# myfavouritekk/vdetlib

Measured on AMD Instinct MI355X. Metric: boxes/sec whole-node (NMS+temporal-conv+link), 300f×10k-box synth; mAP parity, higher is better.
Workload: dtype f32; 1 GPU; configs[1]+[2]: 1 video/GPU, 300 frames x 10000 boxes x 200 classes; per-(frame,class) NMS thresh 0.30 + temporal max-pool w=3 + 3-tap temporal convolution; greedy tubelets: 10 tracks/class (stop < 0.90), IoU-link >= 0.50, spatial max-pool IoU > 0.70 + completion + temporal max-pool; frames=300, boxes=10000, classes=200, scores=rand, parallelism=video-per-gpu x1, 4 distinct videos in flight per GPU

## Files before the change

### vdetlib_amd/csrc/graphlists_kernels.hpp

```cpp
#pragma once
#include <hip/hip_runtime.h>
#include <stdint.h>

#include "nms_kernels.hpp"

namespace vdet {

__device__ __forceinline__ int qreach_slot(const GroupDesc &gd, int g) { return ((gd.box_off >> 8) + g) * 4; }

__global__ __launch_bounds__(256) void row_classes_kernel(const float4 *__restrict__ xbox, const GroupDesc *__restrict__ groups,
                                                          const uint32_t *__restrict__ group_flags, float one_minus_t,
                                                          uint16_t *__restrict__ rowperm, float *__restrict__ qreach)
{
    __shared__ float sw[256];
    __shared__ float sreach[256];
    const int g = blockIdx.x, t = blockIdx.y, tid = threadIdx.x;
    if (!(group_flags[g] & kFlagRegular)) return;
    const GroupDesc gd = groups[g];
    if (t * 256 >= gd.nbox) return;
    const int s = t * 256 + tid;
    const bool valid = s < gd.nbox;
    float wd = 3.0e38f, reach = -3.0e38f;
    if (valid) { const float4 b = xbox[gd.box_off + s]; wd = b.z - b.x; reach = b.x + one_minus_t * ((b.z - b.x) + 1.0f) * 1.001f + 1.0f; }
    sw[tid] = wd;
    __syncthreads();
    int rank = 0;
    for (int j = 0; j < 256; ++j) { const float o = sw[j]; rank += (o < wd || (o == wd && j < tid)) ? 1 : 0; }
    if (valid) rowperm[gd.box_off + t * 256 + rank] = (uint16_t)s;
    sreach[rank] = reach;
    __syncthreads();
    float rc = sreach[tid];
#pragma unroll
    for (int d = 32; d > 0; d >>= 1) rc = fmaxf(rc, __shfl_xor(rc, d, 64));
    if ((tid & 63) == 0) qreach[qreach_slot(gd, g) + 4 * t + (tid >> 6)] = rc;
}

struct ListItem { int32_t group; int32_t tq; };

struct GraphListsParams {
    const float4 *xbox;
    const uint16_t *xord;
    const GroupDesc *groups;
    const uint32_t *group_flags;
    const ListItem *items;
    int nitems;
    float t32, one_minus_t;
    uint32_t *row_deg;
    const float2 *reach_table;
    const uint16_t *rowperm;
    const float *qreach;
    uint16_t *adj;
    uint32_t slot_cap;
    int *status;
    int over_bits;
    uint32_t trash_off;
};

__device__ __forceinline__ void emit_half(uint16_t *__restrict__ adj, uint32_t h, uint32_t boff, const uint16_t *ids, uint32_t *lpos,
                                          const uint16_t myid)
{
    constexpr int kSlots = 4;
    if (__ballot(h != 0u) == 0ull) return;
    uint32_t hk[kSlots];
    uint16_t ek[kSlots];
    int bk[kSlots];
#pragma unroll
    for (int k = 0; k < kSlots; ++k) { hk[k] = h; bk[k] = __builtin_ctz(h) & 31; h &= h - 1u; }
#pragma unroll
    for (int k = 0; k < kSlots; ++k) ek[k] = ids[bk[k]];
#pragma unroll
    for (int k = 0; k < kSlots; ++k) {
        if (hk[k] != 0u) {
            *reinterpret_cast<uint16_t *>(reinterpret_cast<char *>(adj) + (boff + 2u * k)) = ek[k];
            const uint32_t o = __hip_atomic_fetch_add(&lpos[bk[k]], 2u, __ATOMIC_RELAXED, __HIP_MEMORY_SCOPE_WAVEFRONT);
            *reinterpret_cast<uint16_t *>(reinterpret_cast<char *>(adj) + o) = myid;
        }
    }
    boff += 2u * kSlots;
    while (__ballot(h != 0u) != 0ull) {
        if (h != 0u) {
            const int b = __builtin_ctz(h);
            *reinterpret_cast<uint16_t *>(reinterpret_cast<char *>(adj) + boff) = ids[b];
            const uint32_t o = __hip_atomic_fetch_add(&lpos[b], 2u, __ATOMIC_RELAXED, __HIP_MEMORY_SCOPE_WAVEFRONT);
            *reinterpret_cast<uint16_t *>(reinterpret_cast<char *>(adj) + o) = myid;
            boff += 2u;
            h &= h - 1u;
        }
    }
}

__device__ __forceinline__ void emit_block(const uint32_t slot_cap, uint16_t *__restrict__ adj, int *__restrict__ status, const int over_bits,
                                           const uint32_t trash_off, unsigned long long m, const uint32_t tcnt, const uint32_t pat,
                                           const uint32_t ptat, const uint32_t row_slot, const uint32_t col_slot, const uint16_t *cids,
                                           const uint16_t myid, uint32_t *lpos, const int lane)
{
    const uint32_t cnt = (uint32_t)__popcll(m);
    const bool rover = pat + cnt > slot_cap, cover = ptat + tcnt > slot_cap;
    if ((rover && cnt) || (cover && tcnt)) atomicOr(status, over_bits);
    lpos[lane] = cover ? trash_off : (col_slot * slot_cap + ptat) * 2u;
    const uint32_t boff = rover ? trash_off : (row_slot * slot_cap + pat) * 2u;
    emit_half(adj, (uint32_t)m, boff, cids, lpos, myid);
    emit_half(adj, (uint32_t)(m >> 32), boff + 2u * (uint32_t)__popc((uint32_t)m), cids + 32, lpos + 32, myid);
}

template <bool XS, bool INTS>
__device__ __forceinline__ void margin_block(const float4 brx, const float rarea, const float4 *sb, const float *sa, float t32, float t_lo,
                                             uint32_t &lo, uint32_t &hi, bool &anyb)
{
    uint32_t nr0 = 0, nq0 = 0, nr1 = 0, nq1 = 0;
#pragma unroll 1
    for (int g = 0; g < 4; ++g) {
#pragma unroll
        for (int j = 0; j < 8; ++j) {
            const int k = 31 - 8 * g - j;
            float mr, mq;
            pred_margins<XS, INTS>(brx, rarea, sb[k], sa[k], t32, t_lo, mr, mq);
            shl1_or_sign(nr0, mr); shl1_or_sign(nq0, mq);
        }
    }
#pragma unroll 1
    for (int g = 0; g < 4; ++g) {
#pragma unroll
        for (int j = 0; j < 8; ++j) {
            const int k = 31 - 8 * g - j;
            float mr, mq;
            pred_margins<XS, INTS>(brx, rarea, sb[32 + k], sa[32 + k], t32, t_lo, mr, mq);
            shl1_or_sign(nr1, mr); shl1_or_sign(nq1, mq);
        }
    }
    lo = ~nr0; hi = ~nr1;
    anyb = (nr0 != nq0) | (nr1 != nq1);
}

__global__ __launch_bounds__(64, 6) void graph_lists_kernel(const GraphListsParams prm)
{
    __shared__ float4 sbox[2][64];
    __shared__ float sarea[2][64];
    __shared__ uint16_t scord[2][64];
    __shared__ uint32_t lpos[64];
    const int per = gridDim.x >> 3;
    const int idx = (blockIdx.x & 7) * per + (blockIdx.x >> 3);
    if (idx >= prm.nitems) return;
    const ListItem it = prm.items[idx];
    const uint32_t gf = prm.group_flags[it.group];
    if (!(gf & kFlagRegular)) return;
    const GroupDesc gd = prm.groups[it.group];
    const int B = gd.nbox, W = (B + 63) >> 6;
    const int lane = threadIdx.x;
    const int mt = it.tq >> 2, qd = it.tq & 3;
    const int s = mt * 256 + qd * 64 + lane;
    const int v = s < B ? (int)prm.rowperm[gd.box_off + s] : B;
    const unsigned long long rowvalid = __ballot(v < B);
    if (rowvalid == 0ull) return;
    const float my_reach = prm.qreach[qreach_slot(gd, it.group) + it.tq];
    const float2 *rtab = prm.reach_table + reach_slot(gd, it.group);
    const float4 *xb = prm.xbox + gd.box_off;
    const uint16_t *xo = prm.xord + gd.box_off;
    const float t32 = prm.t32;
    const float t_lo = t32 * (1.0f - 4.76837158203125e-7f);
    const TransposeConsts tcs = transpose_consts(lane);
    const bool ints = (gf & kFlagU16) != 0u;
    const uint32_t slot_cap = prm.slot_cap;
    uint16_t *adj = prm.adj;

    float4 br = make_float4(0.f, 0.f, 0.f, 0.f);
    uint16_t myid = 0;
    if (v < B) { br = xb[v]; myid = xo[v]; }
    const float rarea = box_area(br);
    float4 brx = br;
    if (ints) { brx.z += 1.0f; brx.w += 1.0f; }

    int c = mt * 4;
    {
        const int u = c * 64 + lane;
        float4 bc = make_float4(0.f, 0.f, 0.f, 0.f);
        uint16_t oc = 0;
        if (u < B) { bc = xb[u]; oc = xo[u]; }
        sarea[0][lane] = box_area(bc);
        if (ints) { bc.z += 1.0f; bc.w += 1.0f; }
        sbox[0][lane] = bc; scord[0][lane] = oc;
    }
    unsigned long long pm = 0ull;
    uint32_t pat = 0u, ptat = 0u, ptcnt = 0u;
    int pc = -1;
    float fnext = (c + 1 < W) ? rtab[c + 1].y : 3.0e38f;
    for (int buf = 0; c < W; ++c, buf ^= 1) {
        const bool dtile = (c >> 2) == mt;
        const int cn = c + 1;
        bool more = cn < W;
        float4 bn = make_float4(0.f, 0.f, 0.f, 0.f);
        uint16_t on = 0;
        const float fn = __uint_as_float(__builtin_amdgcn_readfirstlane(__float_as_uint(fnext)));
        fnext = (c + 2 < W) ? rtab[c + 2].y : 3.0e38f;
        if (more) {
            more = ((cn >> 2) == mt) || fn <= my_reach;
            const int u = cn * 64 + lane;
            if (more && u < B) { bn = xb[u]; on = xo[u]; }
        }
        const int cols_left = B - c * 64;
        const unsigned long long colvalid = cols_left >= 64 ? ~0ull : ((1ull << cols_left) - 1ull);
        uint32_t lo, hi;
        bool anyb;
        if (ints) { if (!dtile) margin_block<true, true>(brx, rarea, sbox[buf], sarea[buf], t32, t_lo, lo, hi, anyb);
                    else margin_block<false, true>(brx, rarea, sbox[buf], sarea[buf], t32, t_lo, lo, hi, anyb); }
        else { if (!dtile) margin_block<true, false>(brx, rarea, sbox[buf], sarea[buf], t32, t_lo, lo, hi, anyb);
               else margin_block<false, false>(brx, rarea, sbox[buf], sarea[buf], t32, t_lo, lo, hi, anyb); }
        if (__builtin_expect(__ballot(anyb) != 0ull, 0)) {
            lo = hi = 0u;
            for (int k = 0; k < 64; ++k) {
                float4 bk = sbox[buf][k];
                if (ints) { bk.z -= 1.0f; bk.w -= 1.0f; }
                const bool p = pair_pred_exact_slow(br, rarea, bk, sarea[buf][k], t32);
                if (k < 32) lo |= p ? (1u << k) : 0u; else hi |= p ? (1u << (k - 32)) : 0u;
            }
        }
        unsigned long long m = (((unsigned long long)hi << 32) | lo) & colvalid;
        if (dtile) {
            const int d = v - c * 64;
            m &= d < 0 ? ~0ull : (d >= 63 ? 0ull : ~((2ull << d) - 1ull));
        }
        if (v >= B) m = 0ull;
        uint32_t tlo = (uint32_t)m, thi = (uint32_t)(m >> 32);
        wave_transpose64(tlo, thi, tcs);
        if (pc >= 0)
            emit_block(slot_cap, adj, prm.status, prm.over_bits, prm.trash_off, pm, ptcnt, pat, ptat, (uint32_t)(gd.box_off + v),
                       (uint32_t)(gd.box_off + pc * 64 + lane), scord[buf ^ 1], myid, lpos, lane);
        {
            unsigned long long tm = 0ull;
            const int u = c * 64 + lane;
            if (u < B) tm = (((unsigned long long)thi << 32) | tlo) & rowvalid;
            const uint32_t cnt = (uint32_t)__popcll(m), tcnt = (uint32_t)__popcll(tm);
            pat = 0u; ptat = 0u;
            if (cnt) pat = atomicAdd(&prm.row_deg[gd.box_off + v], cnt);
            if (tcnt) ptat = atomicAdd(&prm.row_deg[gd.box_off + u], tcnt);
            pm = m; ptcnt = tcnt; pc = c;
        }
        if (!more) break;
        sarea[buf ^ 1][lane] = box_area(bn);
        if (ints) { bn.z += 1.0f; bn.w += 1.0f; }
        sbox[buf ^ 1][lane] = bn; scord[buf ^ 1][lane] = on;
    }
    if (pc >= 0)
        emit_block(slot_cap, adj, prm.status, prm.over_bits, prm.trash_off, pm, ptcnt, pat, ptat, (uint32_t)(gd.box_off + v),
                   (uint32_t)(gd.box_off + pc * 64 + lane), scord[(pc - mt * 4) & 1], myid, lpos, lane);
}

}
```

### vdetlib_amd/csrc/nms_kernels.hpp

```cpp
#pragma once
#include <hip/hip_runtime.h>
#include <stdint.h>

namespace vdet {

struct GroupDesc {
    int32_t box_off;
    int32_t nbox;
    int64_t bits_off;
};

__device__ __host__ __forceinline__ int64_t bit_word(int nbox, int v, int c)
{
    const int W = (nbox + 63) >> 6;
    return ((int64_t)(v >> 6) * W + c) * 64 + (v & 63);
}
__host__ __device__ __forceinline__ int64_t bit_words_of_group(int nbox)
{
    const int64_t W = (nbox + 63) >> 6;
    return W * W * 64;
}

struct TileDesc {
    int32_t group;
// ... 171 lines not shown
        }
        mn = fminf(mn, b.x); mx = fmaxf(mx, b.x); wm = fmaxf(wm, (b.z - b.x) + 1.0f);
    }
    smin[tid] = mn; smax[tid] = mx; swm[tid] = wm;
    for (int i = tid; i < 257; i += 256) hist[i] = 0;
    __syncthreads();
    for (int d = 128; d > 0; d >>= 1) {
        if (tid < d) { smin[tid] = fminf(smin[tid], smin[tid + d]); smax[tid] = fmaxf(smax[tid], smax[tid + d]); swm[tid] = fmaxf(swm[tid], swm[tid + d]); }
        __syncthreads();
    }
    const float xmin = smin[0], xmax = smax[0];
    const float scale = xmax > xmin ? 256.0f / (xmax - xmin) : 0.0f;
    for (int r = tid; r < B; r += 256) atomicAdd(&hist[xbucket(fb[r].x, xmin, scale) + 1], 1u);
    __syncthreads();
    if (tid == 0) {
        uint32_t run = 0;
        for (int k = 0; k <= 256; ++k) { run += hist[k]; cum[(int64_t)f * 257 + k] = run; }
        info[f * 4 + 0] = xmin; info[f * 4 + 1] = scale; info[f * 4 + 2] = swm[0]; info[f * 4 + 3] = 0.0f;
    }
}

__device__ __forceinline__ void xwindow(const FrameIndex &ix, int f, float x1c, float wc, double t, int &r0, int &r1)
{
    const float xmin = ix.info[f * 4 + 0], scale = ix.info[f * 4 + 1], wmax = ix.info[f * 4 + 2];
    const double wj = fmin((double)wmax, (double)wc / t * 1.001);
    const double lo = (double)x1c - (1.0 - t) * wj * 1.001 - 1.0;
    const double hi = (double)x1c + (1.0 - t) * (double)wc * 1.001 + 1.0;
    const int b0 = xbucket((float)fmax(lo, -3.0e38), xmin, scale);
    const int b1 = xbucket((float)fmin(hi, 3.0e38), xmin, scale);
    r0 = (int)ix.cum[(int64_t)f * 257 + b0];
    r1 = (int)ix.cum[(int64_t)f * 257 + b1 + 1];
}

__global__ __launch_bounds__(256) void frame_flags_kernel(const float4 *__restrict__ boxes,
                                                          const GroupDesc *__restrict__ groups,
                                                          uint32_t *__restrict__ group_flags,
                                                          int *__restrict__ n_irregular)
{
    const GroupDesc gd = groups[blockIdx.x];
    int bad = 0, wide = 0;
    const float inf = __uint_as_float(0x7F800000u);
    for (int v = threadIdx.x; v < gd.nbox; v += 256) {
        const float4 b = boxes[gd.box_off + v];
        const float w = (b.z - b.x) + 1.0f, h = (b.w - b.y) + 1.0f;
        const float a = w * h;
        const bool ok = fabsf(b.x) < inf && fabsf(b.y) < inf && fabsf(b.z) < inf && fabsf(b.w) < inf &&
                        w > 0.0f && h > 0.0f && a < inf;
        bad |= ok ? 0 : 1;
        const bool small = b.x == truncf(b.x) && b.y == truncf(b.y) && b.z == truncf(b.z) && b.w == truncf(b.w) &&
                           fmaxf(fmaxf(b.x, b.y), fmaxf(b.z, b.w)) <= 65535.0f &&
                           ((__float_as_uint(b.x) | __float_as_uint(b.y) | __float_as_uint(b.z) | __float_as_uint(b.w)) >> 31) == 0u;
        wide |= small ? 0 : 1;
    }
    const int any_bad = __syncthreads_or(bad);
    const int any_wide = __syncthreads_or(wide);
    if (threadIdx.x == 0) {
        group_flags[blockIdx.x] = (any_bad ? 0u : kFlagRegular) | (any_wide ? 0u : kFlagU16);
        if (any_bad) atomicAdd(n_irregular, 1);
    }
}

__device__ __attribute__((noinline)) bool pair_pred_exact_slow(float4 bi, float iarea, float4 bj, float jarea, float t32)
{
    return (pair_pred(bi, iarea, bj, jarea, t32) & 1u) != 0;
}

struct TilePair {
    int32_t group;
    int16_t rt, ct;
};

__device__ __forceinline__ float amax(float a, float b) { float r; asm("v_max_f32 %0, %1, %2" : "=v"(r) : "v"(a), "v"(b)); return r; }
__device__ __forceinline__ float amin(float a, float b) { float r; asm("v_min_f32 %0, %1, %2" : "=v"(r) : "v"(a), "v"(b)); return r; }

template <bool XSORTED = false>
__device__ __forceinline__ bool pred_regular(float4 br, float rarea, float4 bc, float carea, float t32, float t32e,
                                             bool &border)
{
    const float xx1 = XSORTED ? bc.x : amax(br.x, bc.x);
    const float yy1 = amax(br.y, bc.y);
    const float xx2 = amin(br.z, bc.z);
    const float yy2 = amin(br.w, bc.w);
    const float w = amax(0.0f, (xx2 - xx1) + 1.0f);
    const float h = (yy2 - yy1) + 1.0f;
    const float inter = w * h;
    const float uni = (rarea + carea) - inter;
    const float r = __builtin_fmaf(-t32, uni, inter);
    const float bnd = t32e * uni;
    const bool p = r >= 0.0f;
    border = !p && (r >= -bnd);
    return p;
}

template <bool XSORTED, bool INTS>
__device__ __forceinline__ void pred_margins(float4 br, float rarea, float4 bc, float carea, float t32, float t_lo, float &r, float &q)
{
    const float xx1 = XSORTED ? bc.x : amax(br.x, bc.x);
    const float yy1 = amax(br.y, bc.y);
    const float xx2 = amin(br.z, bc.z);
    const float yy2 = amin(br.w, bc.w);
    const float w = INTS ? amax(0.0f, xx2 - xx1) : amax(0.0f, (xx2 - xx1) + 1.0f);
    const float h = INTS ? yy2 - yy1 : (yy2 - yy1) + 1.0f;
    const float inter = w * h;
    const float uni = (rarea + carea) - inter;
    r = __builtin_fmaf(-t32, uni, inter);
    q = __builtin_fmaf(-t_lo, uni, inter);
}

__device__ __forceinline__ void shl1_or_sign(uint32_t &acc, float v)
{
    acc = __builtin_amdgcn_alignbit(acc, __float_as_uint(v), 31);
}

struct TransposeConsts {
    uint32_t sel16, sel8;
    uint32_t sh4, m4, sh2, m2, sh1, m1;
};

__device__ __forceinline__ TransposeConsts transpose_consts(int lane)
{
    TransposeConsts t;
    t.sel16 = (lane & 16) ? 0x03020706u : 0x01000504u;
    t.sel8 = (lane & 8) ? 0x03070105u : 0x06020400u;
    t.sh4 = (lane & 4) ? 4u : 28u;  t.m4 = (lane & 4) ? 0xF0F0F0F0u : 0x0F0F0F0Fu;
    t.sh2 = (lane & 2) ? 2u : 30u;  t.m2 = (lane & 2) ? 0xCCCCCCCCu : 0x33333333u;
    t.sh1 = (lane & 1) ? 1u : 31u;  t.m1 = (lane & 1) ? 0xAAAAAAAAu : 0x55555555u;
    return t;
}

__device__ __forceinline__ uint32_t transpose_stage_small(uint32_t r, uint32_t partner, uint32_t sh, uint32_t m)
{
    const uint32_t rot = __builtin_amdgcn_alignbit(partner, partner, sh);
    return (r & m) | (rot & ~m);
}

__device__ __forceinline__ void wave_transpose64(uint32_t &lo, uint32_t &hi, const TransposeConsts &t)
{
    {
        const auto r = __builtin_amdgcn_permlane32_swap(lo, hi, false, false);
        lo = r[0]; hi = r[1];
    }
    {
        auto a = __builtin_amdgcn_permlane16_swap(lo, lo, false, false);
        lo = __builtin_amdgcn_perm(a[0], a[1], t.sel16);
// ... 44 lines not shown
{
    const unsigned long long m = __ballot(p);
    unsigned long long carry_out;
    asm("v_addc_co_u32_e64 %0, %1, %0, %0, %2" : "+v"(acc), "=s"(carry_out) : "s"(m));
}

__device__ __forceinline__ int reach_slot(const GroupDesc &gd, int g) { return (gd.box_off >> 6) + g; }

__global__ __launch_bounds__(256) void reach_table_kernel(const float4 *__restrict__ xbox, const GroupDesc *__restrict__ groups,
                                                          const uint32_t *__restrict__ group_flags, float one_minus_t,
                                                          float2 *__restrict__ table)
{
    const int g = blockIdx.x;
    if (!(group_flags[g] & kFlagRegular)) return;
    const GroupDesc gd = groups[g];
    const int B = gd.nbox, W = (B + 63) >> 6;
    const int lane = threadIdx.x & 63;
    for (int r = threadIdx.x >> 6; r < W; r += 4) {
        const int v = r * 64 + lane;
        float4 b = make_float4(0.f, 0.f, 0.f, 0.f);
        if (v < B) b = xbox[gd.box_off + v];
        float reach = v < B ? b.x + one_minus_t * ((b.z - b.x) + 1.0f) * 1.001f + 1.0f : -3.0e38f;
#pragma unroll
        for (int d = 32; d > 0; d >>= 1) reach = fmaxf(reach, __shfl_xor(reach, d, 64));
        const float first = __shfl(b.x, 0, 64);
        if (lane == 0) table[reach_slot(gd, g) + r] = make_float2(reach, first);
    }
}

template <bool WT>
__global__ __launch_bounds__(256) void iou_bits_sym_kernel(const float4 *__restrict__ xbox,
                                                           const GroupDesc *__restrict__ groups,
                                                           const uint32_t *__restrict__ group_flags,
                                                           const TilePair *__restrict__ pairs, float t32, float one_minus_t,
                                                           uint64_t *__restrict__ bits, uint32_t *__restrict__ row_deg,
                                                           const float2 *__restrict__ reach_table)
{
    __shared__ float4 sbox[256];
    __shared__ float sarea[256];
    const TilePair tp = pairs[blockIdx.x];
    if (!(group_flags[tp.group] & kFlagRegular)) return;
    const GroupDesc gd = groups[tp.group];
    const int B = gd.nbox;
    const int tid = threadIdx.x, lane = tid & 63, w = __builtin_amdgcn_readfirstlane(tid >> 6);
    const int r = tp.rt * 4 + w;
    const int v = r * 64 + lane;
    const float2 *rtab = reach_table + reach_slot(gd, tp.group);
    const int W = (B + 63) >> 6;
    const float my_reach = r < W ? rtab[r].x : -3.0e38f;
    if (tp.ct > tp.rt) {
        float tr = -3.0e38f;
        for (int k = 0; k < 4; ++k) if (tp.rt * 4 + k < W) tr = fmaxf(tr, rtab[tp.rt * 4 + k].x);
        if (tp.ct * 4 >= W || rtab[tp.ct * 4].y > tr) return;
    }
    const float t32e = t32 * 4.76837158203125e-7f;
    const float t_lo = t32 * (1.0f - 4.76837158203125e-7f);
    const TransposeConsts tcs = transpose_consts(lane);
    const bool ints = WT && (group_flags[tp.group] & kFlagU16) != 0u;

    float4 br = make_float4(0.f, 0.f, 0.f, 0.f);
    if (v < B) br = xbox[gd.box_off + v];
    const float rarea = box_area(br);
    float4 brx = br;
    if (ints) { brx.z += 1.0f; brx.w += 1.0f; }
    {
        const int u = tp.ct * 256 + tid;
        float4 bc = make_float4(0.f, 0.f, 0.f, 0.f);
        if (u < B) bc = xbox[gd.box_off + u];
        sarea[tid] = box_area(bc);
        if (ints) { bc.z += 1.0f; bc.w += 1.0f; }
        sbox[tid] = bc;
    }
    __syncthreads();
    const int rows_left = B - r * 64;
    const unsigned long long rowvalid = rows_left >= 64 ? ~0ull : (rows_left > 0 ? ((1ull << rows_left) - 1ull) : 0ull);

    uint32_t dsum = 0;
    for (int q = 0; q < 4; ++q) {
        const int c = tp.ct * 4 + q;
        if (c < r) continue;
        const int cols_left = B - c * 64;
        if (cols_left <= 0) break;
        const unsigned long long colvalid = cols_left >= 64 ? ~0ull : ((1ull << cols_left) - 1ull);
        uint32_t lo = 0, hi = 0, tlo = 0, thi = 0;
        if (rows_left <= 0 || (c > r && rtab[c].y > my_reach)) continue;
        {
            bool anyb = false;
            if (WT) {
                uint32_t nr0 = 0, nq0 = 0, nr1 = 0, nq1 = 0;
#define VDET_MARGIN_BLOCK(XS, IN) \
                _Pragma("unroll 1") for (int g = 0; g < 4; ++g) { \
                    _Pragma("unroll") for (int j = 0; j < 8; ++j) { \
                        const int k = 31 - 8 * g - j; \
                        float mr, mq; \
                        pred_margins<XS, IN>(brx, rarea, sbox[q * 64 + k], sarea[q * 64 + k], t32, t_lo, mr, mq); \
                        shl1_or_sign(nr0, mr); shl1_or_sign(nq0, mq); \
                    } \
                } \
                _Pragma("unroll 1") for (int g = 0; g < 4; ++g) { \
                    _Pragma("unroll") for (int j = 0; j < 8; ++j) { \
                        const int k = 31 - 8 * g - j; \
                        float mr, mq; \
                        pred_margins<XS, IN>(brx, rarea, sbox[q * 64 + 32 + k], sarea[q * 64 + 32 + k], t32, t_lo, mr, mq); \
                        shl1_or_sign(nr1, mr); shl1_or_sign(nq1, mq); \
                    } \
                }
                if (ints) { if (c > r) { VDET_MARGIN_BLOCK(true, true) } else { VDET_MARGIN_BLOCK(false, true) } }
                else { if (c > r) { VDET_MARGIN_BLOCK(true, false) } else { VDET_MARGIN_BLOCK(false, false) } }
#undef VDET_MARGIN_BLOCK
                lo = ~nr0; hi = ~nr1;
                anyb = (nr0 != nq0) | (nr1 != nq1);
            } else {
#pragma unroll
            for (int kk = 0; kk < 32; ++kk) {
                const int k = 31 - kk;
                bool border;
                const bool p = pred_regular(br, rarea, sbox[q * 64 + k], sarea[q * 64 + k], t32, t32e, border);
                anyb |= border;
                shl1_or_pred(lo, p);
                if (!WT) {
                    const unsigned long long b = __ballot(p);
                    tlo = (lane == k) ? (uint32_t)b : tlo;
                    thi = (lane == k) ? (uint32_t)(b >> 32) : thi;
                }
            }
#pragma unroll
            for (int kk = 0; kk < 32; ++kk) {
                const int k = 31 - kk;
                bool border;
                const bool p = pred_regular(br, rarea, sbox[q * 64 + 32 + k], sarea[q * 64 + 32 + k], t32, t32e, border);
                anyb |= border;
                shl1_or_pred(hi, p);
                if (!WT) {
                    const unsigned long long b = __ballot(p);
                    tlo = (lane == 32 + k) ? (uint32_t)b : tlo;
                    thi = (lane == 32 + k) ? (uint32_t)(b >> 32) : thi;
                }
            }
            }
            if (__builtin_expect(__ballot(anyb) != 0ull, 0)) {
                lo = hi = tlo = thi = 0;
                for (int k = 0; k < 64; ++k) {
                    float4 bk = sbox[q * 64 + k];
                    if (ints) { bk.z -= 1.0f; bk.w -= 1.0f; }
                    const bool p = pair_pred_exact_slow(br, rarea, bk, sarea[q * 64 + k], t32);
                    if (k < 32) lo |= p ? (1u << k) : 0u; else hi |= p ? (1u << (k - 32)) : 0u;
                    if (!WT) {
                        const unsigned long long b = __ballot(p);
                        if (lane == k) { tlo = (uint32_t)b; thi = (uint32_t)(b >> 32); }
                    }
                }
            }
            if (WT && c > r) {
                tlo = lo; thi = hi;
                wave_transpose64(tlo, thi, tcs);
            }
        }
        unsigned long long m = (((unsigned long long)hi << 32) | lo) & colvalid;
        if (c == r) m &= ~(1ull << lane);
        if (v < B) { bits[gd.bits_off + bit_word(B, v, c)] = m; dsum += (uint32_t)__popcll(m); }
        if (c > r) {
            const int u = c * 64 + lane;
            if (u < B) {
                const unsigned long long tm = (((unsigned long long)thi << 32) | tlo) & rowvalid;
                bits[gd.bits_off + bit_word(B, u, r)] = tm;
                const uint32_t cnt = (uint32_t)__popcll(tm);
                if (cnt) atomicAdd(&row_deg[gd.box_off + u], cnt);
            }
        }
    }
    if (dsum) atomicAdd(&row_deg[gd.box_off + v], dsum);
}

struct WalkMeta {
    float4 box;
    uint4 row;
};

constexpr int kMaxWordRows = 320;
constexpr int kAdjRows = 128;
constexpr int kAdjBatch = 8;
constexpr int kAdjStage = 16384;

template <int ROWS>
// ... 1018 lines not shown
```

### vdetlib_amd/csrc/vdet_capi.hip

```cpp
#include <hip/hip_runtime.h>
#include <atomic>
#include <chrono>

#include <algorithm>
#include <cmath>
#include <cstdarg>
#include <cstdio>
#include <cstdlib>
#include <cstring>
#include <initializer_list>
#include <string>
#include <vector>

#include "../../include/vdet_hip.h"
#include "nms_kernels.hpp"
#include "binsort_kernels.hpp"
#include "small_kernels.hpp"
#include "detnms_kernels.hpp"
#include "fused_kernels.hpp"
#include "adjrows_kernels.hpp"
#include "graphlists_kernels.hpp"
#include "temporal_kernels.hpp"
#include "tubelet_kernels.hpp"
#include "track_kernels.hpp"
// ... 304 lines not shown
}

int video_table(vdet_ctx *c, StagedTab &t, const Videos &vs, const VidDesc **vids)
{
    *vids = nullptr;
    if (vs.V == 1) return VDET_OK;
    const int rc = stage_video_table(c, t, vs);
    if (rc == VDET_OK) *vids = t.dev.as<VidDesc>();
    return rc;
}

bool fits_upto(int64_t limit, std::initializer_list<int64_t> factors)
{
    if (limit < 0) return false;
    bool zero = false;
    for (const int64_t f : factors) {
        if (f < 0) return false;
        if (f == 0) zero = true;
        else limit /= f;
    }
    return zero || limit >= 1;
}

bool fits_below(int64_t limit, std::initializer_list<int64_t> factors) { return fits_upto(limit - 1, factors); }

float thresh_to_f32(double thresh)
{
    if (thresh != thresh) return NAN;
    float f = (float)thresh;
    if ((double)f < thresh) f = nextafterf(f, INFINITY);
    return f;
}

uint32_t pow2ceil(uint32_t x)
{
    uint32_t p = 1;
    while (p < x) p <<= 1;
    return p;
}

int translate_status(vdet_ctx *c, int st)
{
    if (st & kStPoolAsync) return fail(c, VDET_EAGAIN, "adjacency pool overflow in an asynchronous graph build: run the calls again");
    if (st & kStBadOrder) return fail(c, VDET_EINVAL, "a caller-supplied candidate list holds a count or a box index out of range");
    if (st & kStBadAnchor) return fail(c, VDET_EINVAL, "an anchor frame lies outside the video");
    if (st & kStBadPixAnchor) return fail(c, VDET_EINVAL, "track_pixels: an anchor frame outside the video, or an anchor box that is not finite, beyond 2^20, empty or wholly outside the image (the slot is written as an empty one)");
    if (st & kStBadMerge) return fail(c, VDET_EINVAL, "merge 'max': two paired tubelets differ in the frames of their boxes or in their anchor frame");
    if (st & kStBadPropagate) return fail(c, VDET_EINVAL, "propagate_boxes: a keep_cnt outside 0..cap, a keep_idx outside 0..B-1, or a source box that is not finite or beyond 2^20 (the source writes NaN rows)");
    if (st & kStBadKeep) return fail(c, VDET_EINVAL, "nms_tracks: a keep_cnt outside 0..cap or a keep_idx outside 0..B-1 (the entry is skipped)");
    if (st & kStPatchCap) return fail(c, VDET_ECAP, "tubelet_patches: more present tubelet boxes in the frame range than cap (the first cap windows are valid)");
    if (st & kStSvmBad) return fail(c, VDET_EINVAL, "svm_head: a slot row outside shape or a class column outside W (the group is skipped, nothing is written for it)");
    if (st & kStEvalList) return fail(c, VDET_EINVAL, "a keep list holds a NaN score, an increasing score or a count / box index out of range");
    if (st & kStDivZero) return fail(c, VDET_EDIVZERO, "float division (zero union)");
    if (st & kStCap) return fail(c, VDET_ECAP, "more survivors than the output capacity");
    if (st & kStPool) return fail(c, VDET_EHIP, "internal: adjacency pool overflow");
    return VDET_OK;
}

int make_plan(vdet_ctx *c, NmsPlan &pl)
{
    const size_t budget_words = std::max<size_t>(c->bits_budget / 8, 1);
    size_t cur = 0;
    int t0 = 0, p0 = 0, d0 = 0;
    pl.nmax = 0;
    pl.ntot = 0;
    for (size_t g = 0; g < pl.groups.size(); ++g) {
// ... 198 lines not shown
int build_graph(vdet_ctx *c, const float4 *d_boxes, NmsPlan &pl, float t32, double thresh, bool volume)
{
    const float one_minus_t = (float)std::max(0.0, 1.0 - (thresh == thresh ? thresh : 0.0));
    const size_t G = pl.groups.size();
    c->host_groups = &pl.groups;
    c->sym_built = false;
    c->gt32 = t32;
    c->wmeta_built = false;
    c->wmeta16_built = false;
    c->nodes_valid = false;
    HIPCHK(c, c->groups.reserve(G * sizeof(GroupDesc)));
    HIPCHK(c, c->tiles.reserve(std::max<size_t>(pl.tiles.size(), 1) * sizeof(TileDesc)));
    HIPCHK(c, c->bits.reserve(std::max<size_t>(pl.bits_words_max, 1) * 8));
    HIPCHK(c, c->rowz.reserve((size_t)pl.ntot * 4));
    HIPCHK(c, c->rowmeta.reserve((size_t)pl.ntot * 8));
    HIPCHK(c, c->groupz.reserve(G * 4));
    HIPCHK(c, c->gflags.reserve(G * 4));
    HIPCHK(c, c->pairs.reserve(std::max<size_t>(pl.pairs.size(), 1) * sizeof(TilePair)));
    HIPCHK(c, c->ditems.reserve(std::max<size_t>(pl.ditems.size(), 1) * sizeof(ListItem)));
    if (!(volume && c->vplan_valid)) {
        if (!pl.pairs.empty())
            HIPCHK(c, hipMemcpyAsync(c->pairs.p, pl.pairs.data(), pl.pairs.size() * sizeof(TilePair),
                                     hipMemcpyHostToDevice, c->stream));
        if (!pl.ditems.empty())
            HIPCHK(c, hipMemcpyAsync(c->ditems.p, pl.ditems.data(), pl.ditems.size() * sizeof(ListItem),
                                     hipMemcpyHostToDevice, c->stream));
        HIPCHK(c, hipMemcpyAsync(c->groups.p, pl.groups.data(), G * sizeof(GroupDesc), hipMemcpyHostToDevice, c->stream));
        if (!pl.tiles.empty())
            HIPCHK(c, hipMemcpyAsync(c->tiles.p, pl.tiles.data(), pl.tiles.size() * sizeof(TileDesc),
                                     hipMemcpyHostToDevice, c->stream));
        c->vplan_valid = volume;
    }
    auto direct_now = [&]() {
        return c->direct_lists && c->adj_rows && c->wave_transpose && pl.nmax > 384 && t32 > 1e-30f && t32 < INFINITY && !c->force_general &&
               (size_t)8 * pl.nmax + 24 * 1024 <= c->max_lds && ((unsigned long long)pl.ntot + 1ull) * c->direct_cap * 2ull + 512ull <= 0xFFFFFFFFull;
    };
    auto fixed_pool = [&]() { return direct_now() ? (unsigned long long)pl.ntot * c->direct_cap + std::max<unsigned long long>(c->direct_cap, 128) : 0ull; };
    unsigned long long min_pool = fixed_pool() + (unsigned long long)pl.ntot * (direct_now() ? 1 : 32);
    const bool async = volume && c->async_enabled && c->pool_hint > 0;
    if (async) {
        const unsigned long long dyn_hint = c->pool_hint > fixed_pool() ? c->pool_hint - fixed_pool() : 0ull;
        const unsigned long long want = std::max(min_pool, fixed_pool() + dyn_hint + dyn_hint / 2);
        if (c->adj.cap < want * 2) HIPCHK(c, c->adj.reserve((size_t)want * 2 + 4096));
    } else {
        Counters h0;
        HIPCHK(c, hipMemcpyAsync(&h0, c->d_cnt, sizeof h0, hipMemcpyDeviceToHost, c->stream));
        HIPCHK(c, host_sync(c));
        if (h0.status && !c->latched) c->latched = translate_status(c, h0.status);
        if (h0.eindex && !c->latched) c->latched = fail(c, VDET_EINDEX, "list index out of range");
        if (c->adj.cap < min_pool * 2) HIPCHK(c, c->adj.reserve((size_t)min_pool * 2 + 4096));
    }

    for (int attempt = 0; attempt < 3; ++attempt) {
        const bool direct = direct_now();
        min_pool = fixed_pool() + (unsigned long long)pl.ntot * (direct ? 1 : 32);
        if (!async && c->adj.cap < min_pool * 2) HIPCHK(c, c->adj.reserve((size_t)min_pool * 2 + 4096));
        HIPCHK(c, hipMemsetAsync(c->rowz.p, 0, (size_t)pl.ntot * 4, c->stream));
        HIPCHK(c, hipMemsetAsync(c->rowmeta.p, 0, (size_t)pl.ntot * 8, c->stream));
        HIPCHK(c, hipMemsetAsync(c->groupz.p, 0, G * 4, c->stream));
        if (async) {
            hipLaunchKernelGGL(fold_pool_kernel, dim3(1), dim3(1), 0, c->stream, c->d_cnt);
            HIPCHK(c, hipMemsetAsync((char *)c->d_cnt + kPerBuildOff, 0, sizeof(Counters) - kPerBuildOff, c->stream));
        }
        else HIPCHK(c, hipMemsetAsync(c->d_cnt, 0, sizeof(Counters), c->stream));
        c->direct_ntot = direct ? pl.ntot : 0;
        c->direct_fixed = fixed_pool();
        if (direct) hipLaunchKernelGGL(pool_start_kernel, dim3(1), dim3(1), 0, c->stream, &c->d_cnt->pool_used, fixed_pool());
        const int pool_bits = async ? (kStPool | kStPoolAsync) : kStPool;
        const unsigned long long pool_cap = (c->adj.cap - 2048) / 2;
        const bool use_sym = t32 > 1e-30f && t32 < INFINITY && !c->force_general &&
                             (size_t)8 * pl.nmax + 24 * 1024 <= c->max_lds;
        c->sym_built = use_sym;
        c->wmeta_built = use_sym;
        if (c->wmeta_built) HIPCHK(c, c->wmeta.reserve((size_t)pl.ntot * sizeof(WalkMeta)));
        if (c->wmeta_built && c->adj_rows && pl.nmax > 384) HIPCHK(c, c->wmeta16.reserve((size_t)pl.ntot * sizeof(uint4)));
        if (use_sym) {
            {
                StageTimer tm(c, ST_OTHER);
                hipLaunchKernelGGL(frame_flags_kernel, dim3((unsigned)G), dim3(256), 0, c->stream, d_boxes,
                                   c->groups.as<GroupDesc>(), c->gflags.as<uint32_t>(), &c->d_cnt->irregular);
            }
            if (!volume) c->index_valid = false;
            const int rci = build_frame_index(c, d_boxes, pl.ntot, (int64_t)G, pl.nmax);
            if (rci) return rci;
            HIPCHK(c, c->reachtab.reserve((size_t)(pl.ntot / 64 + (int64_t)G + 2) * sizeof(float2)));
            {
                StageTimer tm(c, ST_OTHER);
                hipLaunchKernelGGL(reach_table_kernel, dim3((unsigned)G), dim3(256), 0, c->stream, c->xbox.as<float4>(),
                                   c->groups.as<GroupDesc>(), c->gflags.as<uint32_t>(), one_minus_t, c->reachtab.as<float2>());
                if (direct) {
                    HIPCHK(c, c->rowperm.reserve((size_t)pl.ntot * 2 + 1024));
                    HIPCHK(c, c->qreach.reserve((size_t)(pl.ntot / 256 + (int64_t)G + 2) * 4 * sizeof(float)));
                    hipLaunchKernelGGL(row_classes_kernel, dim3((unsigned)G, (unsigned)((pl.nmax + 255) / 256)), dim3(256), 0, c->stream,
                                       c->xbox.as<float4>(), c->groups.as<GroupDesc>(), c->gflags.as<uint32_t>(), one_minus_t,
                                       c->rowperm.as<uint16_t>(), c->qreach.as<float>());
                }
            }
        } else {
            c->index_valid = false;
        }
        if (direct && !pl.ditems.empty()) {
            StageTimer tm(c, ST_IOU_BITS);
            GraphListsParams gp;
            gp.xbox = c->xbox.as<float4>(); gp.xord = c->xord.as<uint16_t>(); gp.groups = c->groups.as<GroupDesc>();
            gp.group_flags = c->gflags.as<uint32_t>(); gp.items = c->ditems.as<ListItem>(); gp.nitems = (int)pl.ditems.size();
            gp.t32 = t32; gp.one_minus_t = one_minus_t; gp.row_deg = c->rowz.as<uint32_t>(); gp.reach_table = c->reachtab.as<float2>();
            gp.rowperm = c->rowperm.as<uint16_t>(); gp.qreach = c->qreach.as<float>(); gp.adj = c->adj.as<uint16_t>();
            gp.slot_cap = c->direct_cap; gp.status = &c->d_cnt->status; gp.over_bits = pool_bits | kStDirect;
            gp.trash_off = (uint32_t)((unsigned long long)pl.ntot * c->direct_cap * 2ull);
            hipLaunchKernelGGL(graph_lists_kernel, dim3((gp.nitems + 7) & ~7), dim3(64), 0, c->stream, gp);
        }
        for (size_t bi = 0; bi < pl.batch_tiles.size(); ++bi) {
            const auto bt = pl.batch_tiles[bi];
            const auto bp = pl.batch_pairs[bi];
            const int nt = bt.second - bt.first;
            if (nt <= 0) continue;
            uint64_t *bits_b = c->bits.as<uint64_t>();
            if (use_sym && !direct && bp.second > bp.first) {
                StageTimer tm(c, ST_IOU_BITS);
                if (c->wave_transpose)
                    hipLaunchKernelGGL(iou_bits_sym_kernel<true>, dim3(bp.second - bp.first), dim3(256), 0, c->stream,
                                       c->xbox.as<float4>(), c->groups.as<GroupDesc>(), c->gflags.as<uint32_t>(),
                                       c->pairs.as<TilePair>() + bp.first, t32, one_minus_t, bits_b, c->rowz.as<uint32_t>(),
                                       c->reachtab.as<float2>());
                else
                    hipLaunchKernelGGL(iou_bits_sym_kernel<false>, dim3(bp.second - bp.first), dim3(256), 0, c->stream,
                                       c->xbox.as<float4>(), c->groups.as<GroupDesc>(), c->gflags.as<uint32_t>(),
                                       c->pairs.as<TilePair>() + bp.first, t32, one_minus_t, bits_b, c->rowz.as<uint32_t>(),
                                       c->reachtab.as<float2>());
            }
            int splits = 1;
            if (nt < 4 * c->n_cu) {
                int wmax = 1;
                for (int t = bt.first; t < bt.second; ++t)
                    wmax = std::max(wmax, (pl.groups[pl.tiles[t].group].nbox + 63) / 64);
                splits = std::min((4 * c->n_cu + nt - 1) / nt, (wmax + 3) / 4);
                splits = std::max(1, std::min(splits, 65535));
            }
            {
                StageTimer tm(c, ST_IOU_GEN);
                hipLaunchKernelGGL(iou_bits_kernel, dim3(nt, splits), dim3(256), 0, c->stream, d_boxes,
                                   c->groups.as<GroupDesc>(), c->tiles.as<TileDesc>() + bt.first, t32,
                                   bits_b, c->rowz.as<uint32_t>(), c->groupz.as<uint32_t>(),
                                   use_sym ? c->gflags.as<uint32_t>() : (const uint32_t *)nullptr);
            }
            {
                StageTimer tm(c, ST_ADJ);
                const bool k2_tile = pl.nmax <= 384;
                const bool rows_path = use_sym && c->adj_rows && !k2_tile;
                hipLaunchKernelGGL(k2_tile ? adj_build_kernel<kRowsPerTile> : adj_build_kernel<kAdjRows>, dim3(k2_tile ? nt : 2 * nt),
                                   dim3(k2_tile ? kRowsPerTile : kAdjRows), 0, c->stream, d_boxes,
                                   c->groups.as<GroupDesc>(), c->tiles.as<TileDesc>() + bt.first,
                                   bits_b, c->rowz.as<uint32_t>(), c->rowmeta.as<uint2>(),
                                   c->adj.as<uint16_t>(), &c->d_cnt->pool_used, pool_cap,
                                   &c->d_cnt->status, use_sym ? c->gflags.as<uint32_t>() : (const uint32_t *)nullptr,
                                   use_sym ? frame_index_of(c) : FrameIndex{}, one_minus_t,
                                   async ? (kStPool | kStPoolAsync) : kStPool,
                                   c->wmeta_built ? c->wmeta.as<WalkMeta>() : (WalkMeta *)nullptr,
                                   use_sym ? c->reachtab.as<float2>() : (const float2 *)nullptr, rows_path ? 1 : 0);
                if (rows_path && direct) {
                    if (bi == 0)
// ... 756 lines not shown
}

int vdet_reset_stream(vdet_ctx *c)
{
    if (!c) return VDET_EINVAL;
    c->stream = c->own_stream;
    return VDET_OK;
}

const char *vdet_last_error(vdet_ctx *c) { return c ? c->err.c_str() : "null context"; }

int vdet_set_cache(vdet_ctx *c, int enable)
{
    if (!c) return VDET_EINVAL;
    c->cache_enabled = enable != 0;
    c->graph_valid = c->lists_valid = c->index_valid = c->keys_valid = c->nodes_valid = false;
    return VDET_OK;
}

int vdet_invalidate(vdet_ctx *c)
{
    if (!c) return VDET_EINVAL;
    c->graph_valid = c->lists_valid = c->index_valid = c->keys_valid = c->nodes_valid = false;
    return VDET_OK;
}

int vdet_query(vdet_ctx *c, int what)
{
    if (!c) return VDET_EINVAL;
    if (what == 0) return c->atomic_rank ? 1 : 0;
    if (what == 1) return c->n_cu;
    if (what == 2) return c->all_regular ? 1 : 0;
    if (what == 3) return c->wave_transpose ? 1 : 0;
    if (what == 8) return (int)std::min<long long>(c->n_host_syncs, 0x7FFFFFFF);
    if (what == 10) return (int)std::min<long long>(c->tcn_params.uploads, 0x7FFFFFFF);
    if (what == 11) return (int)std::min<long long>(c->anchor_tab.uploads, 0x7FFFFFFF);
    if (what == 12) return c->vpass_last_items;
    if (what == 13) {
        if (c->ctxs_last_videos <= 0 || !c->ctxs_state.p) return -1;
        std::vector<CtxState> h((size_t)c->ctxs_last_videos);
        if (hipMemcpyAsync(h.data(), c->ctxs_state.p, h.size() * sizeof(CtxState), hipMemcpyDeviceToHost, c->stream) != hipSuccess ||
            host_sync(c) != hipSuccess) return VDET_EHIP;
        int reads = 0;
        for (const CtxState &st : h) reads = std::max(reads, st.empty ? 0 : 2 + (int)st.path);
        return reads;
    }
    if (what == 14) return c->sq_last_path;
    if (what == 9) {
        if (!c->last_sort_binned || !c->sortctl.p) return -1;
        BinSortCtl h{};
        if (hipMemcpyAsync(&h, c->sortctl.p, sizeof h, hipMemcpyDeviceToHost, c->stream) != hipSuccess || host_sync(c) != hipSuccess) return VDET_EHIP;
        return h.nfail;
    }
    if (what >= 4 && what <= 7) {
        unsigned int h[4] = {0, 0, 0, 0};
        if (!c->linkstats.p) return 0;
        if (hipMemcpyAsync(h, c->linkstats.p, 16, hipMemcpyDeviceToHost, c->stream) != hipSuccess ||
            host_sync(c) != hipSuccess) return VDET_EHIP;
        return (int)std::min<unsigned int>(h[what - 4], 0x7FFFFFFFu);
    }
    return VDET_EINVAL;
}

int vdet_set_timing(vdet_ctx *c, int enable)
{
    if (!c) return VDET_EINVAL;
// ... 2889 lines not shown
```

Baseline: 346.1 million boxes/s.

## Replace dual-margin IoU test with single half-gap-shifted sign test

The IoU threshold predicate used to compute two FMA margins per pair (at t and at a slightly lower t) and fell back to a slow exact per-pair loop whenever they disagreed. It now computes one margin shifted by half an ulp-gap of the threshold, which yields the exact decision without the fallback path or the second margin. Coordinate validity is restricted to a bounded range and the threshold is checked for a normal half-gap so the single-FMA rounding argument holds. This removes ALU work and a ballot per block in the hot IoU-bits and graph-lists kernels, and raises the occupancy hint for graph_lists_kernel. The risk is parity: correctness now rests on the rounding argument holding across all inputs.

```diff
diff --git a/vdetlib_amd/csrc/graphlists_kernels.hpp b/vdetlib_amd/csrc/graphlists_kernels.hpp
--- a/vdetlib_amd/csrc/graphlists_kernels.hpp
+++ b/vdetlib_amd/csrc/graphlists_kernels.hpp
@@ -44,7 +44,7 @@
     const uint32_t *group_flags;
     const ListItem *items;
     int nitems;
-    float t32, one_minus_t;
+    float t32, hg, one_minus_t;
     uint32_t *row_deg;
     const float2 *reach_table;
     const uint16_t *rowperm;
@@ -65,7 +65,7 @@
     uint16_t ek[kSlots];
     int bk[kSlots];
 #pragma unroll
-    for (int k = 0; k < kSlots; ++k) { hk[k] = h; bk[k] = __builtin_ctz(h) & 31; h &= h - 1u; }
+    for (int k = 0; k < kSlots; ++k) { hk[k] = h; bk[k] = __builtin_ctz(h | 0x80000000u); h &= h - 1u; }
 #pragma unroll
     for (int k = 0; k < kSlots; ++k) ek[k] = ids[bk[k]];
 #pragma unroll
@@ -104,18 +104,16 @@
 }
 
 template <bool XS, bool INTS>
-__device__ __forceinline__ void margin_block(const float4 brx, const float rarea, const float4 *sb, const float *sa, float t32, float t_lo,
-                                             uint32_t &lo, uint32_t &hi, bool &anyb)
-{
-    uint32_t nr0 = 0, nq0 = 0, nr1 = 0, nq1 = 0;
+__device__ __forceinline__ void margin_block(const float4 brx, const float rarea, const float4 *sb, const float *sa, float t32, float hg,
+                                             uint32_t &lo, uint32_t &hi)
+{
+    uint32_t nr0 = 0, nr1 = 0;
 #pragma unroll 1
     for (int g = 0; g < 4; ++g) {
 #pragma unroll
         for (int j = 0; j < 8; ++j) {
             const int k = 31 - 8 * g - j;
-            float mr, mq;
-            pred_margins<XS, INTS>(brx, rarea, sb[k], sa[k], t32, t_lo, mr, mq);
-            shl1_or_sign(nr0, mr); shl1_or_sign(nq0, mq);
+            shl1_or_sign(nr0, pred_sign<XS, INTS>(brx, rarea, sb[k], sa[k], t32, hg));
         }
     }
 #pragma unroll 1
@@ -123,16 +121,13 @@
 #pragma unroll
         for (int j = 0; j < 8; ++j) {
             const int k = 31 - 8 * g - j;
-            float mr, mq;
-            pred_margins<XS, INTS>(brx, rarea, sb[32 + k], sa[32 + k], t32, t_lo, mr, mq);
-            shl1_or_sign(nr1, mr); shl1_or_sign(nq1, mq);
+            shl1_or_sign(nr1, pred_sign<XS, INTS>(brx, rarea, sb[32 + k], sa[32 + k], t32, hg));
         }
     }
     lo = ~nr0; hi = ~nr1;
-    anyb = (nr0 != nq0) | (nr1 != nq1);
-}
-
-__global__ __launch_bounds__(64, 6) void graph_lists_kernel(const GraphListsParams prm)
+}
+
+__global__ __launch_bounds__(64, 7) void graph_lists_kernel(const GraphListsParams prm)
 {
     __shared__ float4 sbox[2][64];
     __shared__ float sarea[2][64];
@@ -157,7 +152,7 @@
     const float4 *xb = prm.xbox + gd.box_off;
     const uint16_t *xo = prm.xord + gd.box_off;
     const float t32 = prm.t32;
-    const float t_lo = t32 * (1.0f - 4.76837158203125e-7f);
+    const float hg = prm.hg;
     const TransposeConsts tcs = transpose_consts(lane);
     const bool ints = (gf & kFlagU16) != 0u;
     const uint32_t slot_cap = prm.slot_cap;
@@ -200,20 +195,10 @@
         const int cols_left = B - c * 64;
         const unsigned long long colvalid = cols_left >= 64 ? ~0ull : ((1ull << cols_left) - 1ull);
         uint32_t lo, hi;
-        bool anyb;
-        if (ints) { if (!dtile) margin_block<true, true>(brx, rarea, sbox[buf], sarea[buf], t32, t_lo, lo, hi, anyb);
-                    else margin_block<false, true>(brx, rarea, sbox[buf], sarea[buf], t32, t_lo, lo, hi, anyb); }
-        else { if (!dtile) margin_block<true, false>(brx, rarea, sbox[buf], sarea[buf], t32, t_lo, lo, hi, anyb);
-               else margin_block<false, false>(brx, rarea, sbox[buf], sarea[buf], t32, t_lo, lo, hi, anyb); }
-        if (__builtin_expect(__ballot(anyb) != 0ull, 0)) {
-            lo = hi = 0u;
-            for (int k = 0; k < 64; ++k) {
-                float4 bk = sbox[buf][k];
-                if (ints) { bk.z -= 1.0f; bk.w -= 1.0f; }
-                const bool p = pair_pred_exact_slow(br, rarea, bk, sarea[buf][k], t32);
-                if (k < 32) lo |= p ? (1u << k) : 0u; else hi |= p ? (1u << (k - 32)) : 0u;
-            }
-        }
+        if (ints) { if (!dtile) margin_block<true, true>(brx, rarea, sbox[buf], sarea[buf], t32, hg, lo, hi);
+                    else margin_block<false, true>(brx, rarea, sbox[buf], sarea[buf], t32, hg, lo, hi); }
+        else { if (!dtile) margin_block<true, false>(brx, rarea, sbox[buf], sarea[buf], t32, hg, lo, hi);
+               else margin_block<false, false>(brx, rarea, sbox[buf], sarea[buf], t32, hg, lo, hi); }
         unsigned long long m = (((unsigned long long)hi << 32) | lo) & colvalid;
         if (dtile) {
             const int d = v - c * 64;
diff --git a/vdetlib_amd/csrc/nms_kernels.hpp b/vdetlib_amd/csrc/nms_kernels.hpp
--- a/vdetlib_amd/csrc/nms_kernels.hpp
+++ b/vdetlib_amd/csrc/nms_kernels.hpp
@@ -227,6 +227,7 @@
     r1 = (int)ix.cum[(int64_t)f * 257 + b1 + 1];
 }
 
+constexpr float kRegularCoordMax = 1152921504606846976.0f;
 __global__ __launch_bounds__(256) void frame_flags_kernel(const float4 *__restrict__ boxes,
                                                           const GroupDesc *__restrict__ groups,
                                                           uint32_t *__restrict__ group_flags,
@@ -239,8 +240,8 @@
         const float4 b = boxes[gd.box_off + v];
         const float w = (b.z - b.x) + 1.0f, h = (b.w - b.y) + 1.0f;
         const float a = w * h;
-        const bool ok = fabsf(b.x) < inf && fabsf(b.y) < inf && fabsf(b.z) < inf && fabsf(b.w) < inf &&
-                        w > 0.0f && h > 0.0f && a < inf;
+        const bool ok = fabsf(b.x) <= kRegularCoordMax && fabsf(b.y) <= kRegularCoordMax && fabsf(b.z) <= kRegularCoordMax &&
+                        fabsf(b.w) <= kRegularCoordMax && w > 0.0f && h > 0.0f && a < inf;
         bad |= ok ? 0 : 1;
         const bool small = b.x == truncf(b.x) && b.y == truncf(b.y) && b.z == truncf(b.z) && b.w == truncf(b.w) &&
                            fmaxf(fmaxf(b.x, b.y), fmaxf(b.z, b.w)) <= 65535.0f &&
@@ -287,8 +288,13 @@
     return p;
 }
 
+__device__ __forceinline__ void shl1_or_sign(uint32_t &acc, float v)
+{
+    acc = __builtin_amdgcn_alignbit(acc, __float_as_uint(v), 31);
+}
+
 template <bool XSORTED, bool INTS>
-__device__ __forceinline__ void pred_margins(float4 br, float rarea, float4 bc, float carea, float t32, float t_lo, float &r, float &q)
+__device__ __forceinline__ float pred_sign(float4 br, float rarea, float4 bc, float carea, float t32, float hg)
 {
     const float xx1 = XSORTED ? bc.x : amax(br.x, bc.x);
     const float yy1 = amax(br.y, bc.y);
@@ -298,13 +304,7 @@
     const float h = INTS ? yy2 - yy1 : (yy2 - yy1) + 1.0f;
     const float inter = w * h;
     const float uni = (rarea + carea) - inter;
-    r = __builtin_fmaf(-t32, uni, inter);
-    q = __builtin_fmaf(-t_lo, uni, inter);
-}
-
-__device__ __forceinline__ void shl1_or_sign(uint32_t &acc, float v)
-{
-    acc = __builtin_amdgcn_alignbit(acc, __float_as_uint(v), 31);
+    return __builtin_fmaf(hg, uni, __builtin_fmaf(-t32, uni, inter));
 }
 
 struct TransposeConsts {
@@ -415,7 +415,7 @@
 __global__ __launch_bounds__(256) void iou_bits_sym_kernel(const float4 *__restrict__ xbox,
                                                            const GroupDesc *__restrict__ groups,
                                                            const uint32_t *__restrict__ group_flags,
-                                                           const TilePair *__restrict__ pairs, float t32, float one_minus_t,
+                                                           const TilePair *__restrict__ pairs, float t32, float hg, float one_minus_t,
                                                            uint64_t *__restrict__ bits, uint32_t *__restrict__ row_deg,
                                                            const float2 *__restrict__ reach_table)
 {
@@ -437,7 +437,6 @@
         if (tp.ct * 4 >= W || rtab[tp.ct * 4].y > tr) return;
     }
     const float t32e = t32 * 4.76837158203125e-7f;
-    const float t_lo = t32 * (1.0f - 4.76837158203125e-7f);
     const TransposeConsts tcs = transpose_consts(lane);
     const bool ints = WT && (group_flags[tp.group] & kFlagU16) != 0u;
 
@@ -468,32 +467,27 @@
         uint32_t lo = 0, hi = 0, tlo = 0, thi = 0;
         if (rows_left <= 0 || (c > r && rtab[c].y > my_reach)) continue;
         {
-            bool anyb = false;
             if (WT) {
-                uint32_t nr0 = 0, nq0 = 0, nr1 = 0, nq1 = 0;
+                uint32_t nr0 = 0, nr1 = 0;
 #define VDET_MARGIN_BLOCK(XS, IN) \
                 _Pragma("unroll 1") for (int g = 0; g < 4; ++g) { \
                     _Pragma("unroll") for (int j = 0; j < 8; ++j) { \
                         const int k = 31 - 8 * g - j; \
-                        float mr, mq; \
-                        pred_margins<XS, IN>(brx, rarea, sbox[q * 64 + k], sarea[q * 64 + k], t32, t_lo, mr, mq); \
-                        shl1_or_sign(nr0, mr); shl1_or_sign(nq0, mq); \
+                        shl1_or_sign(nr0, pred_sign<XS, IN>(brx, rarea, sbox[q * 64 + k], sarea[q * 64 + k], t32, hg)); \
                     } \
                 } \
                 _Pragma("unroll 1") for (int g = 0; g < 4; ++g) { \
                     _Pragma("unroll") for (int j = 0; j < 8; ++j) { \
                         const int k = 31 - 8 * g - j; \
-                        float mr, mq; \
-                        pred_margins<XS, IN>(brx, rarea, sbox[q * 64 + 32 + k], sarea[q * 64 + 32 + k], t32, t_lo, mr, mq); \
-                        shl1_or_sign(nr1, mr); shl1_or_sign(nq1, mq); \
+                        shl1_or_sign(nr1, pred_sign<XS, IN>(brx, rarea, sbox[q * 64 + 32 + k], sarea[q * 64 + 32 + k], t32, hg)); \
                     } \
                 }
                 if (ints) { if (c > r) { VDET_MARGIN_BLOCK(true, true) } else { VDET_MARGIN_BLOCK(false, true) } }
                 else { if (c > r) { VDET_MARGIN_BLOCK(true, false) } else { VDET_MARGIN_BLOCK(false, false) } }
 #undef VDET_MARGIN_BLOCK
                 lo = ~nr0; hi = ~nr1;
-                anyb = (nr0 != nq0) | (nr1 != nq1);
             } else {
+            bool anyb = false;
 #pragma unroll
             for (int kk = 0; kk < 32; ++kk) {
                 const int k = 31 - kk;
@@ -520,19 +514,15 @@
                     thi = (lane == 32 + k) ? (uint32_t)(b >> 32) : thi;
                 }
             }
-            }
             if (__builtin_expect(__ballot(anyb) != 0ull, 0)) {
                 lo = hi = tlo = thi = 0;
                 for (int k = 0; k < 64; ++k) {
-                    float4 bk = sbox[q * 64 + k];
-                    if (ints) { bk.z -= 1.0f; bk.w -= 1.0f; }
-                    const bool p = pair_pred_exact_slow(br, rarea, bk, sarea[q * 64 + k], t32);
+                    const bool p = pair_pred_exact_slow(br, rarea, sbox[q * 64 + k], sarea[q * 64 + k], t32);
                     if (k < 32) lo |= p ? (1u << k) : 0u; else hi |= p ? (1u << (k - 32)) : 0u;
-                    if (!WT) {
-                        const unsigned long long b = __ballot(p);
-                        if (lane == k) { tlo = (uint32_t)b; thi = (uint32_t)(b >> 32); }
-                    }
+                    const unsigned long long b = __ballot(p);
+                    if (lane == k) { tlo = (uint32_t)b; thi = (uint32_t)(b >> 32); }
                 }
+            }
             }
             if (WT && c > r) {
                 tlo = lo; thi = hi;
diff --git a/vdetlib_amd/csrc/vdet_capi.hip b/vdetlib_amd/csrc/vdet_capi.hip
--- a/vdetlib_amd/csrc/vdet_capi.hip
+++ b/vdetlib_amd/csrc/vdet_capi.hip
@@ -360,6 +360,10 @@
     return f;
 }
 
+float half_gap(float t32) { return (t32 - nextafterf(t32, 0.0f)) * 0.5f; }
+
+bool sym_threshold_ok(float t32) { return t32 > 1e-30f && t32 <= 16777216.0f && std::isnormal(half_gap(t32)); }
+
 uint32_t pow2ceil(uint32_t x)
 {
     uint32_t p = 1;
@@ -624,7 +628,7 @@
         c->vplan_valid = volume;
     }
     auto direct_now = [&]() {
-        return c->direct_lists && c->adj_rows && c->wave_transpose && pl.nmax > 384 && t32 > 1e-30f && t32 < INFINITY && !c->force_general &&
+        return c->direct_lists && c->adj_rows && c->wave_transpose && pl.nmax > 384 && sym_threshold_ok(t32) && !c->force_general &&
                (size_t)8 * pl.nmax + 24 * 1024 <= c->max_lds && ((unsigned long long)pl.ntot + 1ull) * c->direct_cap * 2ull + 512ull <= 0xFFFFFFFFull;
     };
     auto fixed_pool = [&]() { return direct_now() ? (unsigned long long)pl.ntot * c->direct_cap + std::max<unsigned long long>(c->direct_cap, 128) : 0ull; };
@@ -660,7 +664,7 @@
         if (direct) hipLaunchKernelGGL(pool_start_kernel, dim3(1), dim3(1), 0, c->stream, &c->d_cnt->pool_used, fixed_pool());
         const int pool_bits = async ? (kStPool | kStPoolAsync) : kStPool;
         const unsigned long long pool_cap = (c->adj.cap - 2048) / 2;
-        const bool use_sym = t32 > 1e-30f && t32 < INFINITY && !c->force_general &&
+        const bool use_sym = sym_threshold_ok(t32) && !c->force_general &&
                              (size_t)8 * pl.nmax + 24 * 1024 <= c->max_lds;
         c->sym_built = use_sym;
         c->wmeta_built = use_sym;
@@ -696,7 +700,7 @@
             GraphListsParams gp;
             gp.xbox = c->xbox.as<float4>(); gp.xord = c->xord.as<uint16_t>(); gp.groups = c->groups.as<GroupDesc>();
             gp.group_flags = c->gflags.as<uint32_t>(); gp.items = c->ditems.as<ListItem>(); gp.nitems = (int)pl.ditems.size();
-            gp.t32 = t32; gp.one_minus_t = one_minus_t; gp.row_deg = c->rowz.as<uint32_t>(); gp.reach_table = c->reachtab.as<float2>();
+            gp.t32 = t32; gp.hg = half_gap(t32); gp.one_minus_t = one_minus_t; gp.row_deg = c->rowz.as<uint32_t>(); gp.reach_table = c->reachtab.as<float2>();
             gp.rowperm = c->rowperm.as<uint16_t>(); gp.qreach = c->qreach.as<float>(); gp.adj = c->adj.as<uint16_t>();
             gp.slot_cap = c->direct_cap; gp.status = &c->d_cnt->status; gp.over_bits = pool_bits | kStDirect;
             gp.trash_off = (uint32_t)((unsigned long long)pl.ntot * c->direct_cap * 2ull);
@@ -713,12 +717,12 @@
                 if (c->wave_transpose)
                     hipLaunchKernelGGL(iou_bits_sym_kernel<true>, dim3(bp.second - bp.first), dim3(256), 0, c->stream,
                                        c->xbox.as<float4>(), c->groups.as<GroupDesc>(), c->gflags.as<uint32_t>(),
-                                       c->pairs.as<TilePair>() + bp.first, t32, one_minus_t, bits_b, c->rowz.as<uint32_t>(),
+                                       c->pairs.as<TilePair>() + bp.first, t32, half_gap(t32), one_minus_t, bits_b, c->rowz.as<uint32_t>(),
                                        c->reachtab.as<float2>());
                 else
                     hipLaunchKernelGGL(iou_bits_sym_kernel<false>, dim3(bp.second - bp.first), dim3(256), 0, c->stream,
                                        c->xbox.as<float4>(), c->groups.as<GroupDesc>(), c->gflags.as<uint32_t>(),
-                                       c->pairs.as<TilePair>() + bp.first, t32, one_minus_t, bits_b, c->rowz.as<uint32_t>(),
+                                       c->pairs.as<TilePair>() + bp.first, t32, half_gap(t32), one_minus_t, bits_b, c->rowz.as<uint32_t>(),
                                        c->reachtab.as<float2>());
             }
             int splits = 1;
@@ -1541,6 +1545,7 @@
     if (what == 1) return c->n_cu;
     if (what == 2) return c->all_regular ? 1 : 0;
     if (what == 3) return c->wave_transpose ? 1 : 0;
+    if (what == 15) return c->direct_ntot > 0 ? 1 : 0;
     if (what == 8) return (int)std::min<long long>(c->n_host_syncs, 0x7FFFFFFF);
     if (what == 10) return (int)std::min<long long>(c->tcn_params.uploads, 0x7FFFFFFF);
     if (what == 11) return (int)std::min<long long>(c->anchor_tab.uploads, 0x7FFFFFFF);
```

Result: faster. 351.2 million boxes/s (median of 6 runs) (+1.5%).
